# Gifted-s/velarixdb

Measured on AMD Instinct MI355X. Metric: Bloom build keys/s (device-resident keys, bit-exact SipHash-1-3 filter), higher is better.
Workload: dtype u64

## Files before the change

velarixdb_amd/csrc/vbf_partition.hip:

```cpp
#include "vbf_partition.hpp"
#include "vbf_tile_pack.hpp"
#include "vbf_tile_pack_rk.hpp"

namespace vbf {


__global__ __launch_bounds__(256) void k_transpose_u16(const uint16_t* in, uint16_t* out, uint32_t rows,
                                                       uint32_t cols) {
    __shared__ uint16_t t[64][65];
    const uint32_t c0 = blockIdx.x * 64, r0 = blockIdx.y * 64;
    const uint32_t tx = threadIdx.x & 63, ty = threadIdx.x >> 6;
    for (uint32_t y = ty; y < 64; y += 4) {
        const uint32_t r = r0 + y, c = c0 + tx;
        if (r < rows && c < cols) t[y][tx] = in[(uint64_t)r * cols + c];
    }
    __syncthreads();
    for (uint32_t y = ty; y < 64; y += 4) {
        const uint32_t c = c0 + y, r = r0 + tx;
        if (r < rows && c < cols) out[(uint64_t)c * rows + r] = t[tx][y];
    }
}

void launch_transpose_u16(const uint16_t* in, uint16_t* out, uint32_t rows, uint32_t cols, hipStream_t s) {
    hipLaunchKernelGGL(k_transpose_u16, dim3((cols + 63) / 64, (rows + 63) / 64), dim3(256), 0, s, in, out, rows, cols);
}

__global__ __launch_bounds__(256) void k_transpose_u16_v(const uint16_t* in, uint16_t* out, uint32_t rows,
                                                         uint32_t cols, uint32_t in_stride, uint32_t out_stride) {
    __shared__ uint32_t t[64 * 33];
    const uint32_t c0 = blockIdx.x * 64, r0 = blockIdx.y * 64, tid = threadIdx.x;
#pragma unroll
    for (uint32_t q = tid; q < 512; q += 256) {
        const uint32_t r = q >> 3, cv = (q & 7) * 8;
        if (r0 + r < rows && c0 + cv < cols) {
            const uint4 v = *reinterpret_cast<const uint4*>(in + (uint64_t)(r0 + r) * in_stride + c0 + cv);
            uint32_t* d = t + r * 33 + cv / 2;
            d[0] = v.x;
            d[1] = v.y;
            d[2] = v.z;
            d[3] = v.w;
        }
    }
    __syncthreads();
    const uint16_t* t16 = reinterpret_cast<const uint16_t*>(t);
#pragma unroll
    for (uint32_t q = tid; q < 512; q += 256) {
        const uint32_t c = q >> 3, rv = (q & 7) * 8;
        if (c0 + c < cols && r0 + rv < rows) {
            uint32_t w[4];
#pragma unroll
            for (int i = 0; i < 4; ++i)
                w[i] = (uint32_t)t16[(rv + 2 * i) * 66 + c] | ((uint32_t)t16[(rv + 2 * i + 1) * 66 + c] << 16);
            *reinterpret_cast<uint4*>(out + (uint64_t)(c0 + c) * out_stride + r0 + rv) = make_uint4(w[0], w[1], w[2], w[3]);
        }
    }
}

__global__ __launch_bounds__(256) void k_transpose_u16_s(const uint16_t* in, uint16_t* out, uint32_t rows,
                                                         uint32_t cols, uint32_t in_stride, uint32_t out_stride) {
    __shared__ uint16_t t[64][65];
    const uint32_t c0 = blockIdx.x * 64, r0 = blockIdx.y * 64;
    const uint32_t tx = threadIdx.x & 63, ty = threadIdx.x >> 6;
    for (uint32_t y = ty; y < 64; y += 4) {
        const uint32_t r = r0 + y, c = c0 + tx;
        if (r < rows && c < cols) t[y][tx] = in[(uint64_t)r * in_stride + c];
    }
    __syncthreads();
    for (uint32_t y = ty; y < 64; y += 4) {
        const uint32_t c = c0 + y, r = r0 + tx;
        if (r < rows && c < cols) out[(uint64_t)c * out_stride + r] = t[tx][y];
    }
}

hipError_t launch_transpose_u16_strided(const uint16_t* in, uint16_t* out, uint32_t rows, uint32_t cols,
                                        uint32_t in_stride, uint32_t out_stride, hipStream_t s) {
    if (rows == 0 || cols == 0) return hipSuccess;
    if (in_stride < cols || out_stride < rows) return hipErrorInvalidValue;
    const bool vec = in_stride % 8 == 0 && out_stride % 8 == 0 && (reinterpret_cast<uintptr_t>(in) & 15) == 0 &&
                     (reinterpret_cast<uintptr_t>(out) & 15) == 0;
    const dim3 grid((cols + 63) / 64, (rows + 63) / 64);
    if (vec)
        hipLaunchKernelGGL(k_transpose_u16_v, grid, dim3(256), 0, s, in, out, rows, cols, in_stride, out_stride);
    else
        hipLaunchKernelGGL(k_transpose_u16_s, grid, dim3(256), 0, s, in, out, rows, cols, in_stride, out_stride);
    return hipGetLastError();
}

__device__ __forceinline__ void or_group(uint32_t* bitmap, uint4 l, uint32_t nib, uint32_t a, uint32_t b,
                                         uint32_t abl = 0) {
    if (abl == 3) {
        if ((l.x ^ l.y ^ l.z ^ l.w ^ nib) == 0x12345678u && b == 9) bitmap[0] = a;
        return;
    }
    const uint32_t w[4] = {l.x, l.y, l.z, l.w};
#pragma unroll
    for (int c = 0; c < 8; ++c) {
        if ((uint32_t)c >= a && (uint32_t)c < b) {
            const uint32_t idx = ((w[c >> 1] >> ((c & 1) * 16)) & 0xFFFFu) | (((nib >> (4 * c)) & 15u) << 16);
            atomicOr(&bitmap[idx >> 5], 1u << (idx & 31));
        }
    }
}

__device__ __forceinline__ void load_group(const uint32_t* tile, uint32_t g, uint4& l, uint32_t& nib) {
    __builtin_memcpy(&l, tile + g * kGroupWords, 16);
    nib = tile[g * kGroupWords + 4];
}

__device__ __forceinline__ uint32_t group_range(uint32_t gi, uint32_t st, uint32_t en) {
    if (gi * 8 >= en || gi * 8 + 8 <= st) return 0u;
    const uint32_t a = gi * 8 < st ? st - gi * 8 : 0u, b = std::min<uint32_t>(8, en - gi * 8);
    return a | (b << 4);
}

template <int V, int BS = kPBlock, int NG = 8, int LPR = 8>
__global__ __launch_bounds__(BS) void k_seg_or(const uint32_t* tiles, const uint16_t* endsT,
                                                    uint32_t ntiles, PartPlan pl, bool atomic_merge,
                                                    uint32_t* words) {
    __shared__ __attribute__((aligned(16))) uint32_t bitmap[kSegWords];
    constexpr bool MK = V == 7;
    __shared__ __attribute__((aligned(16))) uint32_t marks[BS / 64][MK ? NG * 16 : 1];
    __shared__ __attribute__((aligned(16))) uint2 rinfo[BS / 64][MK ? 64 : 1];
    uint32_t seg, part, parts;
    if (blockIdx.x < pl.nfull) {
        const uint32_t nwg = pl.nfull, q = nwg / 8, r8 = nwg % 8, xcd = blockIdx.x % 8;
        seg = (xcd < r8 ? xcd * (q + 1) : r8 * (q + 1) + (xcd - r8) * q) + blockIdx.x / 8;
        part = 0;
        parts = 1;
    } else {
        const uint32_t r = blockIdx.x - pl.nfull;
        seg = pl.nfull + r / pl.P;
        part = r % pl.P;
        parts = pl.P;
    }
    const uint32_t tid = threadIdx.x, lane = tid & 63, wave = tid >> 6;
    const uint64_t wbase = (uint64_t)seg * kSegWords;
    const uint32_t wn = (uint32_t)std::min<uint64_t>(kSegWords, pl.nwords - wbase);
    const bool own = parts == 1 && !atomic_merge;
    for (uint32_t w = tid * 4; w < kSegWords; w += BS * 4) {
        uint4 v = make_uint4(0, 0, 0, 0);
        if (own && !pl.fresh && pl.ablate < 6) {
            if (w + 4 <= wn)
                v = *reinterpret_cast<const uint4*>(words + wbase + w);
            else if (w < wn) {
                v.x = words[wbase + w];
                if (w + 1 < wn) v.y = words[wbase + w + 1];
                if (w + 2 < wn) v.z = words[wbase + w + 2];
            }
        }
        *reinterpret_cast<uint4*>(bitmap + w) = v;
    }
    __syncthreads();

    const uint32_t t_lo = (uint32_t)((uint64_t)part * ntiles / parts);
    const uint32_t t_hi = (uint32_t)((uint64_t)(part + 1) * ntiles / parts);
    const uint16_t* row_end = endsT + (uint64_t)seg * pl.ntS;
    const uint16_t* row_beg = seg ? endsT + (uint64_t)(seg - 1) * pl.ntS : nullptr;
    static_assert(LPR == 4 || LPR == 8, "lanes per run");
    constexpr uint32_t RPW = 64 / LPR;
    static_assert(V != 3 || RPW * NG <= 64, "one coalesced bounds load per batch covers 64 tiles");
    static_assert(V != 0 || LPR == 8, "the two-stage loop deals 8-lane groups");
    const uint32_t grp = lane / LPR, q8 = lane % LPR;
    const uint32_t step = (BS / 64) * RPW * NG;
    uint32_t tg = t_lo + wave * RPW * NG;
    const uint32_t abl = VBF_ABLATION_BUILD ? pl.ablate : 0u;
    auto tail = [&](uint32_t t, uint32_t st, uint32_t en) {
        const uint32_t* tile = tiles + (uint64_t)t * pl.tile_words;
#pragma unroll 1
        for (uint32_t gi = (st >> 3) + q8 + LPR; gi * 8 < en; gi += LPR) {
            uint4 lt;
            uint32_t nt;
            load_group(tile, gi, lt, nt);
            const uint32_t ab = group_range(gi, st, en);
            or_group(bitmap, lt, nt, ab & 15u, ab >> 4);
        }
    };
    auto spans_more = [](uint32_t st, uint32_t en) { return en > st && ((en + 7) >> 3) - (st >> 3) > LPR; };
    auto lb = [&](uint32_t t0) -> uint32_t {
        const uint32_t t = t0 + lane;
        uint32_t v = 0;
        if (t < t_hi) v = (row_beg ? (uint32_t)row_beg[t] : 0u) | ((uint32_t)row_end[t] << 16);
        return v;
    };

    if (pl.ablate >= 5) {
    } else if constexpr (V == 6 || V == 7) {
        const uint32_t wstep = (BS / 64) * 64;
        struct FB {
            uint32_t v, excl, total;
            uint4 l[NG];
            uint32_t nib[NG], ab[NG];
        };
        auto prep = [&](uint32_t v, FB& b) {
            const uint32_t st = v & 0xFFFFu, en = v >> 16;
            const uint32_t ch = en > st ? ((en + 7) >> 3) - (st >> 3) : 0u;
            uint32_t incl = ch;
            if constexpr (MK) {
                incl = wave_incl_scan_dpp(ch);
                b.total = (uint32_t)__builtin_amdgcn_readlane((int)incl, 63);
            } else {
#pragma unroll
                for (int o = 1; o < 64; o <<= 1) {
                    const uint32_t y = __shfl_up(incl, o);
                    if (lane >= (uint32_t)o) incl += y;
                }
                b.total = (uint32_t)__shfl((int)incl, 63);
            }
            b.v = v;
            b.excl = incl - ch;
        };
        auto locate = [&](const FB& b, uint32_t t0, uint32_t c, const uint32_t*& tile, uint32_t& gi) -> uint32_t {
            uint32_t r = 0;
#pragma unroll
            for (int sft = 32; sft; sft >>= 1)
                if ((uint32_t)__shfl((int)b.excl, (int)r + sft) <= c) r += sft;
            const uint32_t rv = (uint32_t)__shfl((int)b.v, (int)r), rex = (uint32_t)__shfl((int)b.excl, (int)r);
            const uint32_t rst = rv & 0xFFFFu, ren = rv >> 16;
            tile = tiles + (uint64_t)std::min(t0 + r, t_hi - 1) * pl.tile_words;
            gi = (rst >> 3) + (c - rex);
            return c < b.total ? group_range(gi, rst, ren) : 0u;
        };
        auto issue = [&](uint32_t t0, FB& b) {
            if constexpr (MK) {
                rinfo[wave][lane] = make_uint2(b.v, b.excl);
                run_marks_set<NG>(marks[wave], (b.v >> 16) > (b.v & 0xFFFFu), b.excl, lane);
                uint32_t carry = 0;
#pragma unroll
                for (int q = 0; q < NG; ++q) {
                    const uint32_t c = (uint32_t)q * 64 + lane;
                    const uint32_t r1 = run_marks_find(marks[wave], c, carry);
                    b.ab[q] = 0;
                    if (c < b.total) {
                        const uint2 ri = rinfo[wave][r1 - 1];
                        const uint32_t rst = ri.x & 0xFFFFu, ren = ri.x >> 16;
                        const uint32_t gi = (rst >> 3) + (c - ri.y);
                        b.ab[q] = group_range(gi, rst, ren);
                        load_group(tiles + (uint64_t)std::min(t0 + r1 - 1, t_hi - 1) * pl.tile_words, gi, b.l[q],
                                   b.nib[q]);
                    }
                }
            } else {
#pragma unroll
                for (int q = 0; q < NG; ++q) {
                    const uint32_t* tile;
                    uint32_t gi;
                    b.ab[q] = locate(b, t0, (uint32_t)q * 64 + lane, tile, gi);
                    if (b.ab[q]) load_group(tile, gi, b.l[q], b.nib[q]);
                }
            }
        };
        auto consume = [&](uint32_t t0, const FB& b) {
#pragma unroll
            for (int q = 0; q < NG; ++q)
                if (b.ab[q]) or_group(bitmap, b.l[q], b.nib[q], b.ab[q] & 15u, b.ab[q] >> 4, abl);
#pragma unroll 1
            for (uint32_t c0 = 64 * NG; c0 < b.total; c0 += 64) {
                const uint32_t* tile;
                uint32_t gi;
                const uint32_t ab = locate(b, t0, c0 + lane, tile, gi);
                if (ab) {
                    uint4 lt;
                    uint32_t nt;
                    load_group(tile, gi, lt, nt);
                    or_group(bitmap, lt, nt, ab & 15u, ab >> 4, abl);
                }
            }
        };
        uint32_t t0 = t_lo + wave * 64;
        FB A, B;
        uint32_t v1 = lb(t0 + wstep);
        prep(lb(t0), A);
        if (t0 < t_hi) issue(t0, A);
        while (t0 < t_hi) {
            prep(v1, B);
            uint32_t v2 = lb(t0 + 2 * wstep);
            const bool more = t0 + wstep < t_hi;
            if (more) issue(t0 + wstep, B);
            consume(t0, A);
            t0 += wstep;
            if (!more) break;
            prep(v2, A);
            v1 = lb(t0 + 2 * wstep);
            const bool more2 = t0 + wstep < t_hi;
            if (more2) issue(t0 + wstep, A);
            consume(t0, B);
            t0 += wstep;
            if (!more2) break;
        }
    } else if constexpr (V == 3) {
        struct Batch {
            uint32_t be[NG];
            uint4 l[NG];
            uint32_t nib[NG];
        };
        auto spread = [&](uint32_t v, Batch& b) {
#pragma unroll
            for (int g = 0; g < NG; ++g) b.be[g] = (uint32_t)__shfl((int)v, g * RPW + grp);
        };
        auto issue = [&](uint32_t t0, Batch& b) {
#pragma unroll
            for (int g = 0; g < NG; ++g) {
                const uint32_t st = b.be[g] & 0xFFFFu, en = b.be[g] >> 16;
                const uint32_t t = std::min(t0 + g * RPW + grp, t_hi - 1);
                const uint32_t gi = ((st >> 3) + q8) * 8 < en ? (st >> 3) + q8 : st >> 3;
                if (VBF_ABLATION_BUILD && pl.ablate == 4) {
                    b.l[g] = make_uint4(t * 2654435761u + g, lane * 40503u, t ^ lane, gi * 977u);
                    b.nib[g] = t + lane;
                } else {
                    load_group(tiles + (uint64_t)t * pl.tile_words, gi, b.l[g], b.nib[g]);
                }
            }
        };
        auto consume = [&](uint32_t t0, const Batch& b) {
#pragma unroll
            for (int g = 0; g < NG; ++g) {
                const uint32_t st = b.be[g] & 0xFFFFu, en = b.be[g] >> 16;
                const uint32_t ab = group_range((st >> 3) + q8, st, en);
                if (ab) or_group(bitmap, b.l[g], b.nib[g], ab & 15u, ab >> 4, abl);
            }
#pragma unroll
            for (int g = 0; g < NG; ++g) {
                const uint32_t st = b.be[g] & 0xFFFFu, en = b.be[g] >> 16;
                if (spans_more(st, en)) tail(t0 + g * RPW + grp, st, en);
            }
        };
        Batch A, B;
        uint32_t v0 = lb(tg), v1 = lb(tg + step);
        spread(v0, A);
        if (tg < t_hi) issue(tg, A);
        while (tg < t_hi) {
            spread(v1, B);
            uint32_t v2 = lb(tg + 2 * step);
            const bool more = tg + step < t_hi;
            if (more) issue(tg + step, B);
            consume(tg, A);
            tg += step;
            if (!more) break;
            v1 = v2;
            spread(v1, A);
            v2 = lb(tg + 2 * step);
            const bool more2 = tg + step < t_hi;
            if (more2) issue(tg + step, A);
            consume(tg, B);
            tg += step;
            if (!more2) break;
            v1 = v2;
        }
    } else {
        auto bounds = [&](uint32_t t0, uint32_t (&st)[8], uint32_t (&en)[8]) {
#pragma unroll
            for (int g = 0; g < 8; ++g) {
                const uint32_t t = t0 + g * 8 + grp;
                uint32_t b = 0, e = 0;
                if (t < t_hi) {
                    b = row_beg ? row_beg[t] : 0;
                    e = row_end[t];
                }
                st[g] = b;
                en[g] = e;
            }
        };
        uint32_t st[8], en[8];
        bounds(tg, st, en);
        while (tg < t_hi) {
            uint32_t nib[8], ab[8];
            uint4 l[8];
#pragma unroll
            for (int g = 0; g < 8; ++g) {
                const uint32_t gi = (st[g] >> 3) + q8;
                ab[g] = group_range(gi, st[g], en[g]);
                if (ab[g]) {
                    const uint32_t* tile = tiles + (uint64_t)(tg + g * 8 + grp) * pl.tile_words;
                    load_group(tile, gi, l[g], nib[g]);
                }
            }
            const uint32_t tn = tg + step;
            uint32_t st2[8], en2[8];
            bounds(tn, st2, en2);
#pragma unroll
            for (int g = 0; g < 8; ++g)
                if (ab[g]) or_group(bitmap, l[g], nib[g], ab[g] & 15u, ab[g] >> 4, abl);
#pragma unroll
            for (int g = 0; g < 8; ++g)
                if (spans_more(st[g], en[g])) tail(tg + g * 8 + grp, st[g], en[g]);
#pragma unroll
            for (int g = 0; g < 8; ++g) {
                st[g] = st2[g];
                en[g] = en2[g];
            }
            tg = tn;
        }
    }
    __syncthreads();
    if (pl.ablate == 7) return;
    if (own) {
        for (uint32_t w = tid * 4; w < wn; w += BS * 4) {
            if (w + 4 <= wn)
                *reinterpret_cast<uint4*>(words + wbase + w) = *reinterpret_cast<const uint4*>(bitmap + w);
            else
                for (uint32_t x = w; x < wn; ++x) words[wbase + x] = bitmap[x];
        }
    } else {
        for (uint32_t w = tid; w < wn; w += BS) {
            const uint32_t v = bitmap[w];
            if (v) atomicOr(words + wbase + w, v);
        }
    }
}

static PartPlan make_plan(uint32_t m, uint32_t k, bool fixed = true, bool lp = true, int group_sb = 0, bool pu = false) {
    PartPlan pl{};
    const bool group = group_sb != 0;
    const int sb = group ? group_sb : kSegBits;
    pl.k = k;
    pl.m = m;
    pl.mu = ~0ull / m;
    pl.nwords = ((uint64_t)m + 31) / 32;
    pl.nseg = (uint32_t)(((uint64_t)m + (1u << sb) - 1) >> sb);
    pl.nseg_pad = (pl.nseg + 3) & ~3u;
    const bool ck = k == 4 || k == 9 || k == 10 || k == 19;
    static const int kcls = [] { const char* e = getenv("VBF_KCLASS"); return e ? atoi(e) : 1; }();
    pl.kc = (!ck && kcls != 0) ? tile_pack_class(k) : 0u;
    pl.lp = lp ? 1u : 0u;
    static const int k1env = [] { const char* e = getenv("VBF_K1"); return e ? atoi(e) : -1; }();
    pl.k1v = (uint32_t)((k1env >= 0 ? k1env == 1 : true) && (k == 10 || k == 19) && pl.nseg <= 4 * 512);
    if (pl.kc) pl.k1v = 1;
    if (group) {
        pl.kc = 0;
        pl.k1v = 1;
    }
    static const int c16env = [] { const char* e = getenv("VBF_C16"); return e ? atoi(e) : -1; }();
    pl.c16 = (uint32_t)(!group && (k == 19 || k == 4 || k == 10) &&
                        (c16env >= 0 ? c16env != 0 : ((k == 19 && !pl.k1v) || (k == 4 && pl.nseg > 2048))));
    if (!fixed && pl.c16) pl.k1v = 0;
    static const int k14env = [] { const char* e = getenv("VBF_K1_4"); return e ? atoi(e) : 0; }();
    static const int satenv = [] { const char* e = getenv("VBF_SAT"); return e ? atoi(e) : 1; }();
    if (k14env == 1 && satenv != 0 && k == 4 && fixed && lp && m == 0xFFFFFFFFu && !group && pl.c16) pl.k1v = 1;
    if (pu) {
        pl.c16 = 0;
        if (k == 4 && m == 0xFFFFFFFFu) {
            pl.k1v = 0;
        } else if ((k == 4 || k == 9) && kcls != 0) {
            pl.kc = tile_pack_class(k);
            pl.k1v = 1;
        }
    }
    const K1Shape sh = k1_shape((int)(pl.kc ? pl.kc : k), fixed, (int)pl.k1v);
    const uint32_t rmax = (uint32_t)(ck || pl.kc ? sh.rounds : rounds_max((int)k));
    const uint32_t kpr = (uint32_t)sh.bs / (uint32_t)(ck ? sh.spl : 1);
    static const int etenv = [] { const char* e = getenv("VBF_ENDS_T"); return e ? atoi(e) : 1; }();
    pl.ends_t = (uint32_t)(etenv != 0);
    const uint32_t cnt_words = pl.c16 ? ((pl.nseg + 7) & ~7u) / 2 : pl.nseg_pad;
    pl.cnt_words = cnt_words;
    pl.gd_words = group ? (((pl.nseg + 1) / 2 + 3) & ~3u) : 0u;
    for (uint32_t per_cu : {2u, 1u}) {
        const uint32_t budget = kLdsPerCu / per_cu;
        const int64_t avail = (int64_t)budget - 4 * (16 + kLenBuckets) - 4 * (int64_t)cnt_words - 4 * (int64_t)pl.gd_words;
        const int64_t cmax = avail * 2 / 5 - 8 - (group ? 7 * (int64_t)pl.nseg : 0);
        const int64_t kt = std::min<int64_t>((int64_t)rmax * kpr, cmax / k);
        if (kt >= kpr || per_cu == 1) {
            pl.KT = (uint32_t)std::max<int64_t>(kt, 1);
            break;
        }
    }
    pl.R = (pl.KT + kpr - 1) / kpr;
    pl.C = pl.KT * k;
    pl.CP = (pl.C + 7) & ~7u;
    pl.CPg = group ? (pl.C + 7 * pl.nseg + 7) & ~7u : pl.CP;
    pl.tile_words = (group_words(pl.CPg) + 3) & ~3u;
    static const int tpad = [] { const char* e = getenv("VBF_TILE_PAD"); return e ? atoi(e) : 4; }();
    pl.tile_words += (uint32_t)std::max(0, tpad) & ~3u;
    pl.nsegS = (pl.nseg + 7) & ~7u;
    pl.lds1 = (group_words(group ? pl.CPg : pl.CP) + cnt_words + 16 + kLenBuckets + pl.gd_words) * 4;
    static const int lds_min = [] { const char* e = getenv("VBF_TILE_LDS_MIN"); return e ? atoi(e) : 0; }();
    if (lds_min > 0) pl.lds1 = std::max<uint32_t>(pl.lds1, std::min<uint32_t>((uint32_t)lds_min, kLdsPerCu));
    static const int env = [] { const char* e = getenv("VBF_STAGGER"); return e ? atoi(e) : -1; }();
    const uint32_t sleeps = env >= 0 ? (uint32_t)env : 0;
    pl.stagger_lo = 256;
    pl.stagger_hi = 512;
    pl.stagger_sleeps = sleeps;
    static const int abl = [] {
        const char* e = VBF_ABLATION_BUILD ? getenv("VBF_ABLATE") : nullptr;
        return e ? atoi(e) : 0;
    }();
    pl.ablate = (uint32_t)abl;
    static const int k3v = [] { const char* e = getenv("VBF_K3"); return e ? atoi(e) : 0; }();
    pl.k3v = (uint32_t)k3v;
    static const int lord = [] { const char* e = getenv("VBF_LEN_ORDER"); return e ? atoi(e) : 1; }();
    pl.len_order = (uint32_t)(lord != 0 && !group);
    static const int stg = [] { const char* e = getenv("VBF_STAGE_KEYS"); return e ? atoi(e) : 1; }();
    pl.stage_keys = (uint32_t)(stg != 0 && (uint64_t)(pl.KT + 1) / 2 + 2ull * pl.KT <= group_words(pl.CP));
    return pl;
}

bool partition_supported(uint32_t m, uint32_t k) {
    if (m == 0 || k < 1 || k > (uint32_t)kStash) return false;
    for (bool fixed : {true, false})
        for (bool lp : {true, false}) {
            const PartPlan pl = make_plan(m, k, fixed, lp);
            if (pl.lds1 > kLdsPerCu || pl.CP > 65535) return false;
        }
    return true;
}

static uint64_t build_chunk_idx() {
    static const uint64_t v = [] {
        const char* e = getenv("VBF_BUILD_CHUNK_LOG2");
        return e ? 1ull << std::max(20, std::min(33, atoi(e))) : kBuildChunkIdx;
    }();
    return v;
}

uint64_t build_chunk_default() { return build_chunk_idx(); }

static uint64_t chunk_keys_for(const PartPlan& pl, uint64_t n, uint64_t chunk_idx = 0) {
    const uint64_t tiles_per_chunk = std::max<uint64_t>(1, (chunk_idx ? chunk_idx : build_chunk_idx()) / pl.C);
    return std::min<uint64_t>(n, tiles_per_chunk * pl.KT);
}

uint64_t partition_workspace_bytes(uint64_t n, uint32_t m, uint32_t k, uint64_t chunk_idx) {
    if (!partition_supported(m, k)) return 0;
    uint64_t need = 0;
    for (bool fixed : {true, false})
        for (bool lp : {true, false}) {
            const PartPlan pl = make_plan(m, k, fixed, lp);
            const uint64_t ntiles = (chunk_keys_for(pl, n, chunk_idx) + pl.KT - 1) / pl.KT;
            need = std::max<uint64_t>(need,
                                      ntiles * (uint64_t)pl.tile_words * 4 + (ntiles + 8) * (uint64_t)pl.nsegS * 4 + 512);
        }
    return need;
}

bool partition_fresh_ok(uint64_t n, uint32_t m, uint32_t k, uint64_t chunk_idx) {
    if (!partition_supported(m, k) || n == 0) return false;
    for (bool fixed : {true, false})
        for (bool lp : {true, false}) {
            const PartPlan pl = make_plan(m, k, fixed, lp);
            const uint64_t ck = chunk_keys_for(pl, n, chunk_idx);
            const uint64_t ntiles = (ck + pl.KT - 1) / pl.KT;
            const uint32_t G = std::max<uint32_t>(1, std::min<uint32_t>((uint32_t)ntiles, (512 + pl.nseg - 1) / pl.nseg));
            if (ck < n || G > 1) return false;
        }
    return true;
}

bool group_pack_supported(uint64_t m, uint32_t k, int sb) {
    if (m == 0 || m > (2048ull << sb) || m > (1ull << 31) || (k != 10 && k != 19)) return false;
    for (bool fixed : {true, false}) {
        const PartPlan pl = make_plan((uint32_t)m, k, fixed, true, sb);
        if (pl.lds1 > kLdsPerCu / 2 || pl.CPg > 65535 || pl.nseg > 4 * 512) return false;
        if (7ull * pl.nseg * 20 > 9ull * pl.C) return false;
    }
    return true;
}

PartPlan make_group_plan(uint32_t m, uint32_t k, bool fixed, int sb) { return make_plan(m, k, fixed, true, sb); }

PartPlan make_probe_pu_plan(uint32_t m, uint32_t k, bool fixed, bool lp) {
    PartPlan pl = make_plan(m, k, fixed, lp, 0, true);
    pl.stage_keys = 0;
    return pl;
}

uint32_t group_pack_slots(uint32_t k) {
    const K1Shape sh = k1_shape((int)k, true, 1);
    return (uint32_t)(sh.rounds * sh.kl);
}

hipError_t launch_group_pack(const KeyBatch& kb, const DevKeys& dk, const PartPlan& pl, uint32_t ntiles,
                             uint32_t* tiles, uint16_t* endsT, uint16_t* posv, int sb, hipStream_t s) {
    hipError_t err = hipErrorInvalidValue;
    if (!kb.len_prefix || (pl.k != 10 && pl.k != 19) || pl.k1v != 1 || !pl.ends_t) return err;
    if (sb != kByteSegBits && sb != kSegBits) return err;
    with_fmt(pick_fmt(dk.keys, dk.offsets, dk.stride), true, [&]<int FMT, bool LP>() {
        if constexpr (LP) {
            auto fn = sb == kByteSegBits
                          ? (pl.k == 10 ? k_tile_pack<FMT, true, 10, true, false, 1, 0, kByteSegBits, true>
                                        : k_tile_pack<FMT, true, 19, true, false, 1, 0, kByteSegBits, true>)
                          : (pl.k == 10 ? k_tile_pack<FMT, true, 10, true, false, 1, 0, kSegBits, true>
                                        : k_tile_pack<FMT, true, 19, true, false, 1, 0, kSegBits, true>);
            hipFuncAttributes fa{};
            err = hipFuncGetAttributes(&fa, reinterpret_cast<const void*>(fn));
            if (err == hipSuccess && fa.sharedSizeBytes != 0) err = hipErrorInvalidKernelFile;
            if (err == hipSuccess)
                err = hipFuncSetAttribute(reinterpret_cast<const void*>(fn),
                                          hipFuncAttributeMaxDynamicSharedMemorySize, (int)pl.lds1);
            if (err == hipSuccess) {
                hipLaunchKernelGGL(fn, dim3(ntiles), dim3(512), pl.lds1, s, dk, pl, tiles, endsT, posv);
                err = hipGetLastError();
            }
        }
    });
    return err;
}

hipError_t launch_tile_pack_main(int fmt, bool lp, const DevKeys& dk, const PartPlan& pl, uint32_t ntiles,
                                 uint32_t* tiles, uint16_t* ends, hipStream_t s) {
    switch (fmt) {
        case 16: case 32: return launch_tile_pack_main_a(fmt, lp, dk, pl, ntiles, tiles, ends, s);
        case 8: case 24: return launch_tile_pack_main_b(fmt, lp, dk, pl, ntiles, tiles, ends, s);
        default: return launch_tile_pack_main_c(fmt, lp, dk, pl, ntiles, tiles, ends, s);
    }
}

hipError_t launch_build_partitioned(const KeyBatch& kb, uint32_t m, uint32_t k, uint32_t* words,
                                    void* ws, uint64_t ws_bytes, bool atomic_merge, hipStream_t s, bool fresh,
                                    uint64_t chunk_idx) {
    if (kb.n == 0 || k == 0) return hipSuccess;
    if (!partition_supported(m, k)) return hipErrorInvalidValue;
    PartPlan pl = make_plan(m, k, pick_fmt(kb.keys, kb.offsets, kb.stride) > 0, kb.len_prefix);
    const uint64_t chunk_keys = chunk_keys_for(pl, kb.n, chunk_idx);
    const uint64_t max_tiles = (chunk_keys + pl.KT - 1) / pl.KT;
    if (ws_bytes < partition_workspace_bytes(kb.n, m, k, chunk_idx)) return hipErrorInvalidValue;
    uint32_t* tiles = reinterpret_cast<uint32_t*>(ws);
    uint16_t* ends = reinterpret_cast<uint16_t*>(
        (reinterpret_cast<uintptr_t>(tiles + max_tiles * pl.tile_words) + 15) & ~(uintptr_t)15);
    uint16_t* endsT = ends + max_tiles * pl.nsegS;

    for (uint64_t lo = 0; lo < kb.n; lo += chunk_keys) {
        const uint64_t cn = std::min<uint64_t>(chunk_keys, kb.n - lo);
        DevKeys dk{kb.keys, kb.offsets, kb.off_base, kb.stride, cn};
        if (kb.offsets)
            dk.offsets = kb.offsets + lo;
        else
            dk.keys = kb.keys + lo * kb.stride;
        const uint32_t ntiles = (uint32_t)((cn + pl.KT - 1) / pl.KT);
        pl.ntS = (ntiles + 7) & ~7u;
        hipError_t err = hipSuccess;
        phase_begin(kPhaseTileSort, s);
        if (pl.kc) {
            const int fmt = pick_fmt(dk.keys, dk.offsets, dk.stride);
            uint16_t* e = pl.ends_t ? endsT : ends;
            err = pl.kc <= 12 ? (pl.lp ? launch_tile_pack_class_a(fmt, dk, pl, ntiles, tiles, e, s)
                                       : launch_tile_pack_class_c(fmt, dk, pl, ntiles, tiles, e, s))
                              : (pl.lp ? launch_tile_pack_class_b(fmt, dk, pl, ntiles, tiles, e, s)
                                       : launch_tile_pack_class_d(fmt, dk, pl, ntiles, tiles, e, s));
        } else if (kb.len_prefix && m == 0xFFFFFFFFu &&
                   (err = launch_tile_pack_sat(pick_fmt(dk.keys, dk.offsets, dk.stride), dk, pl, ntiles, tiles,
                                               pl.ends_t ? endsT : ends, s)) != hipErrorNotSupported) {
        } else {
            err = launch_tile_pack_main(pick_fmt(dk.keys, dk.offsets, dk.stride), kb.len_prefix, dk, pl, ntiles, tiles,
                                        pl.ends_t ? endsT : ends, s);
        }
        if (err != hipSuccess) return err;
        phase_end(kPhaseTileSort, s);
        if (!pl.ends_t) {
            phase_begin(kPhaseTranspose, s);
            err = launch_transpose_u16_strided(ends, endsT, ntiles, pl.nseg, pl.nsegS, pl.ntS, s);
            if (err != hipSuccess) return err;
            phase_end(kPhaseTranspose, s);
        }
        pl.G = std::max<uint32_t>(1, std::min<uint32_t>(ntiles, (512 + pl.nseg - 1) / pl.nseg));
        const bool merge = atomic_merge || pl.G > 1;
        pl.fresh = (fresh && lo == 0 && !merge) ? 1u : 0u;
        if (fresh && lo == 0 && merge) return hipErrorInvalidValue;
        pl.nfull = pl.G > 1 ? 0u : pl.nseg;
        pl.P = pl.G;
        if (pl.G == 1 && tail_split_enabled()) {
            const uint32_t ncu = device_cu_count(), rem = ncu ? pl.nseg % ncu : 0u;
            if (pl.nseg > ncu && rem > 0 && ncu / rem >= 2) {
                pl.P = std::min<uint32_t>(std::min<uint32_t>(ncu / rem, 16u), ntiles);
                pl.nfull = pl.nseg - rem;
            }
        }
        if (pl.fresh && pl.nfull < pl.nseg) {
            const uint64_t w0 = (uint64_t)pl.nfull * kSegWords;
            err = hipMemsetAsync(words + w0, 0, (pl.nwords - w0) * 4, s);
            if (err != hipSuccess) return err;
        }
        phase_begin(kPhaseSegOr, s);
        const uint32_t k3v = pl.k3v ? pl.k3v : (pl.C / std::max(pl.nseg, 1u) < kShortRun ? 14u : 15u);
        auto k3 = k3v == 14 ? k_seg_or<7, kPBlock, 4>
                : k3v == 15 ? k_seg_or<7, kPBlock, 5>
                : k3v == 16 ? k_seg_or<7, kPBlock, 6>
                : k3v == 13 ? k_seg_or<3, kPBlock, 4, 4>
                : k3v == 10 ? k_seg_or<6, kPBlock, 4>
                : k3v == 11 ? k_seg_or<6, kPBlock, 5>
                : k3v == 12 ? k_seg_or<6, kPBlock, 6>
                : k3v == 8 ? k_seg_or<3, kPBlock, 6>
                : k3v == 3 ? k_seg_or<3, kPBlock, 4>
                : k3v == 5 ? k_seg_or<3, 768, 6>
                : k3v == 6 ? k_seg_or<3, 768, 8>
                : k3v == 1 ? k_seg_or<0>
                           : k_seg_or<3, kPBlock, 5>;
        const int bs = (k3v == 5 || k3v == 6) ? 768 : kPBlock;
        static const uint32_t k3passes = [] {
            const char* e = getenv("VBF_K3_PASSES");
            return (uint32_t)std::max(1, e ? atoi(e) : 1);
        }();
        const uint32_t passes = std::max<uint32_t>(1, std::min<uint32_t>(k3passes, ntiles / std::max<uint32_t>(pl.P, 16)));
        for (uint32_t ps = 0; ps < passes; ++ps) {
            const uint32_t a = (uint32_t)((uint64_t)ntiles * ps / passes), b = (uint32_t)((uint64_t)ntiles * (ps + 1) / passes);
            PartPlan pp = pl;
            if (ps > 0) pp.fresh = 0;
            hipLaunchKernelGGL(k3, dim3(pl.nfull + (pl.nseg - pl.nfull) * pl.P), dim3(bs), 0, s,
                               tiles + (uint64_t)a * pl.tile_words, endsT + a, b - a, pp, merge, words);
        }
        phase_end(kPhaseSegOr, s);
        err = hipGetLastError();
        if (err != hipSuccess) return err;
    }
    return hipSuccess;
}
}
```

Baseline: 25.00 billion.

## Add branchless V8 segment-OR kernel with prefetched bounds and flat masked atomics

Adds a new k_seg_or variant (V==8) and makes it the default for long runs. It prefetches the next tile batch's row bounds one step ahead and clamps tile and group indices so loads happen without branching. It also replaces the per-character conditional atomicOr with an unconditional atomicOr whose bit is masked to zero when out of range. The aim is to remove divergence and expose more memory-level parallelism, at the cost of issuing extra (no-op) LDS atomics for inactive characters.

```diff
diff --git a/velarixdb_amd/csrc/vbf_partition.hip b/velarixdb_amd/csrc/vbf_partition.hip
--- a/velarixdb_amd/csrc/vbf_partition.hip
+++ b/velarixdb_amd/csrc/vbf_partition.hip
@@ -102,6 +102,20 @@
     }
 }
 
+__device__ __forceinline__ void or_group_flat(uint32_t* bitmap, uint4 l, uint32_t nib, uint32_t ab, uint32_t abl = 0) {
+    if (abl == 3) {
+        or_group(bitmap, l, nib, ab & 15u, ab >> 4, abl);
+        return;
+    }
+    const uint32_t mask = ((1u << (ab >> 4)) - 1u) & ~((1u << (ab & 15u)) - 1u);
+    const uint32_t w[4] = {l.x, l.y, l.z, l.w};
+#pragma unroll
+    for (int c = 0; c < 8; ++c) {
+        const uint32_t idx = ((w[c >> 1] >> ((c & 1) * 16)) & 0xFFFFu) | (((nib >> (4 * c)) & kNibMask) << 16);
+        atomicOr(&bitmap[idx >> 5], ((mask >> c) & 1u) << (idx & 31));
+    }
+}
+
 __device__ __forceinline__ void load_group(const uint32_t* tile, uint32_t g, uint4& l, uint32_t& nib) {
     __builtin_memcpy(&l, tile + g * kGroupWords, 16);
     nib = tile[g * kGroupWords + 4];
@@ -110,6 +124,12 @@
 __device__ __forceinline__ uint32_t group_range(uint32_t gi, uint32_t st, uint32_t en) {
     if (gi * 8 >= en || gi * 8 + 8 <= st) return 0u;
     const uint32_t a = gi * 8 < st ? st - gi * 8 : 0u, b = std::min<uint32_t>(8, en - gi * 8);
+    return a | (b << 4);
+}
+
+__device__ __forceinline__ uint32_t group_range_flat(uint32_t gi, uint32_t st, uint32_t en) {
+    const uint32_t lo = gi * 8;
+    const uint32_t a = std::min<uint32_t>(st - std::min(st, lo), 8u), b = std::min<uint32_t>(en - std::min(en, lo), 8u);
     return a | (b << 4);
 }
 
@@ -118,7 +138,7 @@
                                                     uint32_t ntiles, PartPlan pl, bool atomic_merge,
                                                     uint32_t* words) {
     __shared__ __attribute__((aligned(16))) uint32_t bitmap[kSegWords];
-    constexpr bool MK = V == 7;
+    constexpr bool MK = V == 7 || V == 8;
     __shared__ __attribute__((aligned(16))) uint32_t marks[BS / 64][MK ? NG * 16 : 1];
     __shared__ __attribute__((aligned(16))) uint2 rinfo[BS / 64][MK ? 64 : 1];
     uint32_t seg, part, parts;
@@ -184,6 +204,104 @@
     };
 
     if (pl.ablate >= 5) {
+    } else if constexpr (V == 8) {
+        const uint32_t wstep = (BS / 64) * 64;
+        const uint32_t gmax = pl.tile_words / kGroupWords - 1;
+        const uint16_t* rb = endsT + (uint64_t)(seg ? seg - 1 : 0u) * pl.ntS;
+        struct FB {
+            uint32_t v, excl, total;
+            uint4 l[NG];
+            uint32_t nib[NG], ab[NG];
+        };
+        struct Bd {
+            uint32_t beg, end;
+        };
+        auto bounds = [&](uint32_t t0) -> Bd {
+            const uint32_t t = std::min(t0 + lane, t_hi - 1);
+            return Bd{rb[t], row_end[t]};
+        };
+        auto prep = [&](Bd d, uint32_t t0, FB& b) {
+            const bool in = t0 + lane < t_hi;
+            const uint32_t st = (in && seg) ? d.beg : 0u, en = in ? d.end : 0u;
+            const uint32_t ch = en > st ? ((en + 7) >> 3) - (st >> 3) : 0u;
+            const uint32_t incl = wave_incl_scan_dpp(ch);
+            b.total = (uint32_t)__builtin_amdgcn_readlane((int)incl, 63);
+            b.v = st | (en << 16);
+            b.excl = incl - ch;
+        };
+        auto locate = [&](const FB& b, uint32_t t0, uint32_t c, const uint32_t*& tile, uint32_t& gi) -> uint32_t {
+            uint32_t r = 0;
+#pragma unroll
+            for (int sft = 32; sft; sft >>= 1)
+                if ((uint32_t)__shfl((int)b.excl, (int)r + sft) <= c) r += sft;
+            const uint32_t rv = (uint32_t)__shfl((int)b.v, (int)r), rex = (uint32_t)__shfl((int)b.excl, (int)r);
+            const uint32_t rst = rv & 0xFFFFu, ren = rv >> 16;
+            tile = tiles + (uint64_t)std::min(t0 + r, t_hi - 1) * pl.tile_words;
+            gi = (rst >> 3) + (c - rex);
+            return c < b.total ? group_range(gi, rst, ren) : 0u;
+        };
+        auto issue = [&](uint32_t t0, FB& b) {
+            rinfo[wave][lane] = make_uint2(b.v, b.excl);
+            run_marks_set<NG>(marks[wave], (b.v >> 16) > (b.v & 0xFFFFu), b.excl, lane);
+            uint32_t carry = 0;
+            const uint32_t* p = tiles + (uint64_t)std::min(t0 + lane, t_hi - 1) * pl.tile_words;
+#pragma unroll
+            for (int q = 0; q < NG; ++q) {
+                const uint32_t c = (uint32_t)q * 64 + lane;
+                const uint32_t r1 = run_marks_find(marks[wave], c, carry);
+                const bool live = c < b.total;
+                const uint2 ri = rinfo[wave][live ? r1 - 1 : 0u];
+                const uint32_t rst = ri.x & 0xFFFFu, ren = ri.x >> 16;
+                const uint32_t gi = (rst >> 3) + (c - ri.y);
+                b.ab[q] = live ? group_range_flat(gi, rst, ren) : 0u;
+                const uint32_t* pq = tiles + (uint64_t)std::min(t0 + r1 - 1, t_hi - 1) * pl.tile_words +
+                                     std::min(gi, gmax) * kGroupWords;
+                p = live ? pq : p;
+                load_group(p, 0, b.l[q], b.nib[q]);
+            }
+        };
+        auto consume = [&](uint32_t t0, const FB& b) {
+#pragma unroll
+            for (int q = 0; q < NG; ++q) or_group_flat(bitmap, b.l[q], b.nib[q], b.ab[q], abl);
+#pragma unroll 1
+            for (uint32_t c0 = 64 * NG; c0 < b.total; c0 += 64) {
+                const uint32_t* tile;
+                uint32_t gi;
+                const uint32_t ab = locate(b, t0, c0 + lane, tile, gi);
+                if (ab) {
+                    uint4 lt;
+                    uint32_t nt;
+                    load_group(tile, gi, lt, nt);
+                    or_group_flat(bitmap, lt, nt, ab, abl);
+                }
+            }
+        };
+        uint32_t t0 = t_lo + (uint32_t)__builtin_amdgcn_readfirstlane((int)wave) * 64;
+        if (t0 < t_hi) {
+            FB A, B;
+            const Bd d0 = bounds(t0);
+            Bd d1 = bounds(t0 + wstep);
+            prep(d0, t0, A);
+            issue(t0, A);
+            while (t0 + 2 * wstep < t_hi) {
+                prep(d1, t0 + wstep, B);
+                d1 = bounds(t0 + 2 * wstep);
+                issue(t0 + wstep, B);
+                consume(t0, A);
+                prep(d1, t0 + 2 * wstep, A);
+                d1 = bounds(t0 + 3 * wstep);
+                issue(t0 + 2 * wstep, A);
+                consume(t0 + wstep, B);
+                t0 += 2 * wstep;
+            }
+            const bool two = t0 + wstep < t_hi;
+            if (two) {
+                prep(d1, t0 + wstep, B);
+                issue(t0 + wstep, B);
+            }
+            consume(t0, A);
+            if (two) consume(t0 + wstep, B);
+        }
     } else if constexpr (V == 6 || V == 7) {
         const uint32_t wstep = (BS / 64) * 64;
         struct FB {
@@ -669,10 +787,13 @@
             if (err != hipSuccess) return err;
         }
         phase_begin(kPhaseSegOr, s);
-        const uint32_t k3v = pl.k3v ? pl.k3v : (pl.C / std::max(pl.nseg, 1u) < kShortRun ? 14u : 15u);
+        const uint32_t k3v = pl.k3v ? pl.k3v : (pl.C / std::max(pl.nseg, 1u) < kShortRun ? 14u : 18u);
         auto k3 = k3v == 14 ? k_seg_or<7, kPBlock, 4>
                 : k3v == 15 ? k_seg_or<7, kPBlock, 5>
                 : k3v == 16 ? k_seg_or<7, kPBlock, 6>
+                : k3v == 17 ? k_seg_or<8, kPBlock, 4>
+                : k3v == 18 ? k_seg_or<8, kPBlock, 5>
+                : k3v == 19 ? k_seg_or<8, kPBlock, 6>
                 : k3v == 13 ? k_seg_or<3, kPBlock, 4, 4>
                 : k3v == 10 ? k_seg_or<6, kPBlock, 4>
                 : k3v == 11 ? k_seg_or<6, kPBlock, 5>
```

After: 25.18 billion, median of 6. No clear change (+0.7%).
